# jac0626/Neighbor-Aware-Reinforcement-Learning-Fosters-Cooperation-in-Spatial-Public-Goods-Games-

Measured on AMD Instinct MI355X. Metric: agent-steps/sec (L×L×iters×replicas) + achieved HBM GB/s, L=200, higher is better.
Workload: dtype f64

## Files before the change

neighbor-aware-reinforcement-learning-fosters-cooperation-in-spatial-public-goods-games-_amd/csrc/spgg_device.h:

```cpp
#pragma once

#include <hip/hip_runtime.h>

#include <stdint.h>

#include "spgg_abi.h"

namespace spgg {

#ifndef SPGG_BLOCK
#define SPGG_BLOCK 256
#endif
constexpr int kBlock = SPGG_BLOCK;
static_assert(kBlock == 256 || kBlock == 512, "SPGG_BLOCK must be 256 or 512");
constexpr int kWaves = kBlock / 64;

__device__ __forceinline__ int wrap(int x, int L) {
  while (x < 0) x += L;
  while (x >= L) x -= L;
  return x;
}

template <int CTRL>
__device__ __forceinline__ double dpp_f64(double x) {
// ... 50 lines not shown
    constexpr int h = CNT > 1 ? CNT / 2 : 1;
    if constexpr (MASK >= 16) {
      if constexpr (CNT > 1) {
#pragma unroll
        for (int i = 0; i < h; ++i) v[i] = swap_sum<MASK>(v[i], v[i + h]);
      } else {
        v[0] = swap_sum<MASK>(v[0], v[0]);
      }
    } else {
      if constexpr (CNT > 1) {
        const bool upper = (lane & MASK) != 0;
#pragma unroll
        for (int i = 0; i < h; ++i) {
          const T send = upper ? v[i] : v[i + h];
          const T keep = upper ? v[i + h] : v[i];
          v[i] = keep + partner<MASK>(send);
        }
      } else {
        v[0] += partner<MASK>(v[0]);
      }
    }
    transpose_level<(CNT > 1 ? CNT / 2 : 1), MASK / 2, K, T>(v, lane);
  }
}

template <int K>
__device__ __forceinline__ double block_reduce(double (&v)[K], double* lds) {
  static_assert(K >= 1 && K <= 64 && (K & (K - 1)) == 0, "K must be a power of two");
  transpose_level<K, 32, K, double>(v, threadIdx.x & 63);
  const int lane = threadIdx.x & 63, wave = threadIdx.x >> 6;
  constexpr int per = 64 / K;
  if ((lane & (per - 1)) == 0) lds[wave * K + lane / per] = v[0];
  __syncthreads();
  double tot = 0.0;
  if (threadIdx.x < K) {
#pragma unroll
    for (int w = 0; w < kWaves; ++w) tot += lds[w * K + threadIdx.x];
  }
  return tot;
}

__device__ __forceinline__ double uniform_f64(double x) {
  return __hiloint2double(__builtin_amdgcn_readfirstlane(__double2hiint(x)),
                          __builtin_amdgcn_readfirstlane(__double2loint(x)));
}
__device__ __forceinline__ uint64_t uniform_u64(uint64_t x) {
  return (uint64_t)(uint32_t)__builtin_amdgcn_readfirstlane((int)(x >> 32)) << 32 |
         (uint32_t)__builtin_amdgcn_readfirstlane((int)(uint32_t)x);
}

__device__ __forceinline__ double max_f64(double a, double b) {
  double r;
  asm("v_max_f64 %0, %1, %2" : "=v"(r) : "v"(a), "v"(b));
  return r;
}

template <int MASK>
__device__ __forceinline__ double swap_max(double x) {
  const int lo = __double2loint(x), hi = __double2hiint(x);
  const auto l = MASK == 32 ? __builtin_amdgcn_permlane32_swap(lo, lo, false, false)
                            : __builtin_amdgcn_permlane16_swap(lo, lo, false, false);
  const auto h = MASK == 32 ? __builtin_amdgcn_permlane32_swap(hi, hi, false, false)
                            : __builtin_amdgcn_permlane16_swap(hi, hi, false, false);
  return max_f64(__hiloint2double(h[0], l[0]), __hiloint2double(h[1], l[1]));
}

__device__ __forceinline__ double wave_max(double v) {
  v = swap_max<32>(v);
  v = swap_max<16>(v);
  v = max_f64(v, partner<8>(v));
  v = max_f64(v, partner<4>(v));
  v = max_f64(v, partner<2>(v));
  v = max_f64(v, partner<1>(v));
  return v;
}

__device__ __forceinline__ double mt_double(uint32_t a, uint32_t b) {
  return ((double)(a >> 5) * 67108864.0 + (double)(b >> 6)) / 9007199254740992.0;
}

__device__ __forceinline__ uint2 philox2x32_10(uint2 c, uint32_t k) {
#pragma unroll
  for (int r = 0; r < 10; ++r) {
    if (r) k += 0x9E3779B9u;
    const uint64_t p = (uint64_t)0xD256D193u * c.x;
    c = make_uint2((uint32_t)(p >> 32) ^ k ^ c.y, (uint32_t)p);
  }
  return c;
}

__host__ __device__ inline uint64_t u53_threshold(double thr) {
  return (uint64_t)__builtin_ceil(thr * 9007199254740992.0);
}

__device__ __forceinline__ uint2 philox_block(int idx, int t, uint32_t key) {
  return philox2x32_10(make_uint2((uint32_t)idx >> 1, (uint32_t)t), key);
}
__device__ __forceinline__ void philox_decide(uint32_t bits, uint64_t thr53, int* explore, int* rbit) {
  const uint32_t thr31 = (uint32_t)((thr53 + ((1ull << 22) - 1)) >> 22);
  *explore = (bits >> 1) < thr31 ? 1 : 0;
  *rbit = (int)(bits & 1u);
}
__device__ __forceinline__ void philox_draw(int idx, int t, uint32_t key, uint64_t thr53, int* explore,
                                            int* rbit) {
  const uint2 w = philox_block(idx, t, key);
  philox_decide((idx & 1) ? w.y : w.x, thr53, explore, rbit);
// ... 45 lines not shown
```

neighbor-aware-reinforcement-learning-fosters-cooperation-in-spatial-public-goods-games-_amd/csrc/spgg_kernels.hip:

```cpp
#include <hip/hip_runtime.h>

#include <algorithm>
#include <numeric>
#include <type_traits>
#include <cstdio>
#include <cstdlib>
#include <cstring>
#include <new>
#include <string>
#include <thread>
#include <vector>

#include "spgg_abi.h"
#include "spgg_test.h"
#include "spgg_device.h"
#include "spgg_mt.h"
#include "spgg_clusters.h"
#include "spgg_correlations.h"
#include "spgg_reputation.h"

using namespace spgg;

#ifndef SPGG_ABLATE
#define SPGG_ABLATE 0
// ... 340 lines not shown
  __device__ __forceinline__ void store(uint8_t* dst, int pitch, int h, uint8_t* dbit, int tid) {
    const int r0 = tid / DW, col = tid - (tid / DW) * DW;
    const int o0 = r0 * pitch + col * 4;
#pragma unroll
    for (int j = 0; j < J; ++j) {
      if (r0 < RPP && r0 + j * RPP < h) {
        const int o = o0 + j * RPP * pitch;
        *reinterpret_cast<uint32_t*>(dst + o) = buf[j];
        if (dbit) *reinterpret_cast<uint32_t*>(dbit + o) = buf[j] & 0x01010101u;
      }
    }
  }
};

__device__ __forceinline__ void build_plus_counts(uint8_t* pc, const uint8_t* d, int sw, int rows, int tid) {
  const int lane = tid & 63;
  const int wave = __builtin_amdgcn_readfirstlane(tid >> 6);
  for (int y = wave; y < rows; y += kWaves) {
    const uint8_t* p = d + y * sw + lane;
    const int cnt = p[1] + p[sw] + p[sw + 1] + p[sw + 2] + p[2 * sw + 1];
    pc[y * kPcPitch + lane] = (uint8_t)(cnt << 3);
  }
}

template <int DWPR>
__device__ __forceinline__ void build_plus_counts_dw(uint8_t* pc, const uint8_t* dplane, int sw, int rows,
                                                     int soff, int tid) {
  const uint32_t s0 = 8u * soff, s1 = s0 + 8u, s2 = s0 + 16u;
  const int swd = sw >> 2;
  for (int task = tid; task < rows * DWPR; task += kBlock) {
    const int y = task / DWPR, xd = task - (task / DWPR) * DWPR;
    const uint32_t* r0 = reinterpret_cast<const uint32_t*>(dplane) + y * swd + xd;
    const uint32_t a0 = r0[0], a1 = r0[1];
    const uint32_t b0 = r0[swd], b1 = r0[swd + 1];
    const uint32_t c0 = r0[2 * swd], c1 = r0[2 * swd + 1];
    const uint32_t cnt = __builtin_amdgcn_alignbit(a1, a0, s1) + __builtin_amdgcn_alignbit(b1, b0, s0) +
                         __builtin_amdgcn_alignbit(b1, b0, s1) + __builtin_amdgcn_alignbit(b1, b0, s2) +
                         __builtin_amdgcn_alignbit(c1, c0, s1);
    *reinterpret_cast<uint32_t*>(pc + y * kPcPitch + xd * 4) = cnt << 3;
  }
}

__device__ __forceinline__ void build_plus_counts_prev(uint8_t* pc, const uint8_t* s, int sw, int rows, int tid) {
  const int lane = tid & 63;
  const int wave = __builtin_amdgcn_readfirstlane(tid >> 6);
  for (int y = wave; y < rows; y += kWaves) {
    const uint8_t* p = s + y * sw + lane;
    const int cnt = ((p[1] >> 3) & 1) + ((p[sw] >> 3) & 1) + ((p[sw + 1] >> 3) & 1) + ((p[sw + 2] >> 3) & 1) +
                    ((p[2 * sw + 1] >> 3) & 1);
    pc[y * kPcPitch + lane] = (uint8_t)(cnt << 3);
  }
}
template <int DWPR>
__device__ __forceinline__ void build_plus_counts_prev_dw(uint8_t* pc, const uint8_t* splane, int sw, int rows,
                                                          int soff, int tid) {
  const uint32_t s0 = 8u * soff, s1 = s0 + 8u, s2 = s0 + 16u;
  const int swd = sw >> 2;
  constexpr uint32_t kB3 = 0x01010101u;
  for (int task = tid; task < rows * DWPR; task += kBlock) {
    const int y = task / DWPR, xd = task - (task / DWPR) * DWPR;
    const uint32_t* r0 = reinterpret_cast<const uint32_t*>(splane) + y * swd + xd;
    const uint32_t a0 = (r0[0] >> 3) & kB3, a1 = (r0[1] >> 3) & kB3;
    const uint32_t b0 = (r0[swd] >> 3) & kB3, b1 = (r0[swd + 1] >> 3) & kB3;
    const uint32_t c0 = (r0[2 * swd] >> 3) & kB3, c1 = (r0[2 * swd + 1] >> 3) & kB3;
    const uint32_t cnt = __builtin_amdgcn_alignbit(a1, a0, s1) + __builtin_amdgcn_alignbit(b1, b0, s0) +
                         __builtin_amdgcn_alignbit(b1, b0, s1) + __builtin_amdgcn_alignbit(b1, b0, s2) +
                         __builtin_amdgcn_alignbit(c1, c0, s1);
    *reinterpret_cast<uint32_t*>(pc + y * kPcPitch + xd * 4) = cnt << 3;
  }
}

#define T_AT(t, o) (*reinterpret_cast<const double*>((t) + (o)))
__device__ __forceinline__ double payoff_pc(const uint8_t* pc, int ry, int rx, const double* tb, double norm_min,
                                            double norm_den, double norm_rcp) {
  const uint8_t* p = pc + ry * kPcPitch + rx + 1;
  const char* t = reinterpret_cast<const char*>(tb);
  const uint32_t x0 = p[kPcPitch], x1 = p[0], x2 = p[2 * kPcPitch], x3 = p[kPcPitch - 1], x4 = p[kPcPitch + 1];
  double tot = T_AT(t, x0);
  tot = tot + T_AT(t, x1);
  tot = tot + T_AT(t, x2);
  tot = tot + T_AT(t, x3);
  tot = tot + T_AT(t, x4);
  return div_uniform(tot - norm_min, norm_den, norm_rcp);
}

#undef T_AT

__device__ __forceinline__ double rcp_diag(double x) {
  double r = __builtin_amdgcn_rcp(x);
  r = __builtin_fma(r, __builtin_fma(-x, r, 1.0), r);
  r = __builtin_fma(r, __builtin_fma(-x, r, 1.0), r);
  return r;
}

constexpr uint64_t stat_bytes(int a, int b, int c, int d, int e, int f, int g, int h) {
  return (uint64_t)(uint8_t)a | (uint64_t)(uint8_t)b << 8 | (uint64_t)(uint8_t)c << 16 | (uint64_t)(uint8_t)d << 24 |
         (uint64_t)(uint8_t)e << 32 | (uint64_t)(uint8_t)f << 40 | (uint64_t)(uint8_t)g << 48 |
         (uint64_t)(uint8_t)h << 56;
}


enum { ALG_Q = SPGG_ALG_QLEARNING, ALG_SARSA = SPGG_ALG_SARSA, ALG_ES = SPGG_ALG_EXPECTED_SARSA,
       ALG_DQ = SPGG_ALG_DOUBLE_Q };

__device__ __forceinline__ int greedy2(double v0, double v1) { return v0 >= v1 ? 0 : 1; }

__device__ __forceinline__ double mean2(double x, double y) { return (x + y) * 0.5; }

__device__ __forceinline__ double expected_q(double v0, double v1, double eps) {
  const double po = eps * 0.5;
  const double pgr = (1.0 - eps) + po;
  const int g = greedy2(v0, v1);
  return (g == 0 ? pgr : po) * v0 + (g == 1 ? pgr : po) * v1;
}

__device__ __forceinline__ int draw_bit(const TileArgs& a, int rep, int g, int p) {
  const uint32_t w = *at(a.draws, (uint32_t)(rep * a.draw_words + (g >> 5) * a.planes + p));
  return (int)((w >> (g & 31)) & 1u);
}

template <int RNG>
// ... 128 lines not shown
    qb[0] = e == 0 ? nq2 : y0; qb[1] = e == 1 ? nq2 : y1; qb[2] = e == 2 ? nq2 : y2; qb[3] = e == 3 ? nq2 : y3;
    *rn0 = sn ? q[2] : q[0];
    *rn1 = sn ? q[3] : q[1];
    return diag ? diag_td_dq(q, qb, e, sn, rew, pg) : 0.f;
  } else {
    const double o0 = so ? q[2] : q[0], o1 = so ? q[3] : q[1];
    const double v0 = sn ? q[2] : q[0], v1 = sn ? q[3] : q[1];
    const double qc = act ? o1 : o0;
    double target;
    if constexpr (ALG == ALG_Q) {
      target = max_f64(v0, v1);
    } else if constexpr (ALG == ALG_SARSA) {
      int ex, rbt;
      draw_pair<RNG>(a, rep, g, t, key, eps53, 1, &ex, &rbt);
      target = (ex ? rbt : greedy2(v0, v1)) ? v1 : v0;
    } else {
      target = expected_q(v0, v1, eps);
    }
    const double td = (rew + gamma * target) - qc;
    const double q1 = qc + alpha * td;
    const bool s1 = so != 0, a1 = act != 0;
    q[0] = (!s1 && !a1) ? q1 : q[0];
    q[1] = (!s1 && a1) ? q1 : q[1];
    q[2] = (s1 && !a1) ? q1 : q[2];
    q[3] = (s1 && a1) ? q1 : q[3];
    const double w0 = sn ? q[2] : q[0], w1 = sn ? q[3] : q[1];
    *rn0 = w0;
    *rn1 = w1;
    if (!diag) return 0.f;
    double target2;
    if constexpr (ALG == ALG_SARSA) {
      int ex, rbt;
      draw_pair<RNG>(a, rep, g, t, key, eps53, 2, &ex, &rbt);
      target2 = (ex ? rbt : greedy2(w0, w1)) ? w1 : w0;
    } else {
      target2 = ALG == ALG_ES ? expected_q(w0, w1, eps) : max_f64(w0, w1);
    }
    return (float)fabs(pg.diag_alpha * ((rew + dgamma * target2) - q1));
  }
}

template <bool M2>
__device__ __forceinline__ double prev_max_diff(const double* rew, int ca, int w) {
  const double r0 = rew[ca];
  constexpr int KN = M2 ? 12 : 4;
  const int nb[12] = {ca - w, ca + w, ca - 1, ca + 1, ca - 2 * w, ca + 2 * w, ca - 2, ca + 2,
                      ca - w - 1, ca - w + 1, ca + w - 1, ca + w + 1};
  double rw[KN];
#pragma unroll
  for (int k = 0; k < KN; ++k) rw[k] = rew[nb[k]];
  double m = rw[0];
#pragma unroll
  for (int k = 1; k < KN; ++k) m = max_f64(m, rw[k]);
  return max_f64(m - r0, 0.0);
}

template <int ALG, typename PT>
__device__ __forceinline__ float prev_diag_td(const double (&q)[4], const double (&qb)[ALG == ALG_DQ ? 4 : 1],
                                              int e, int sn, double rew, const PT& pg, double eps_prev) {
  if constexpr (ALG == ALG_DQ) {
    return diag_td_dq(q, qb, e, sn, rew, pg);
  } else {
    double w0, w1, o0, o1;
    select_row<0>(q, qb, sn, &w0, &w1);
    select_row<0>(q, qb, e >> 1, &o0, &o1);
    const double q1 = (e & 1) ? o1 : o0;
    const double target2 = ALG == ALG_ES ? expected_q(w0, w1, eps_prev) : max_f64(w0, w1);
    return (float)fabs(pg.diag_alpha * ((rew + pg.diag_gamma * target2) - q1));
  }
}


__device__ __forceinline__ double wave_sum(double v) {
  {
    const int lo = __double2loint(v), hi = __double2hiint(v);
    const auto l = __builtin_amdgcn_permlane32_swap(lo, lo, false, false);
    const auto h = __builtin_amdgcn_permlane32_swap(hi, hi, false, false);
    v = __hiloint2double(h[0], l[0]) + __hiloint2double(h[1], l[1]);
  }
  {
    const int lo = __double2loint(v), hi = __double2hiint(v);
    const auto l = __builtin_amdgcn_permlane16_swap(lo, lo, false, false);
    const auto h = __builtin_amdgcn_permlane16_swap(hi, hi, false, false);
    v = __hiloint2double(h[0], l[0]) + __hiloint2double(h[1], l[1]);
  }
  v += partner<8>(v);
  v += partner<4>(v);
  v += partner<2>(v);
  v += partner<1>(v);
  return v;
}

#ifndef SPGG_BAR_DEBUG
#define SPGG_BAR_DEBUG 0
#endif
constexpr uint32_t kBarrierPolls = 1u << 21;

__device__ __forceinline__ bool replica_barrier(const spgg_impl::PersistArgs& pa, int rep, int tile,
                                                int tiles_per_rep, uint32_t k,
                                                unsigned long long* arrive_stamp = nullptr) {
  __shared__ int bar_ok;
  asm volatile("s_waitcnt vmcnt(0)" ::: "memory");
  __syncthreads();
  if (arrive_stamp && threadIdx.x == 0) *arrive_stamp = __builtin_amdgcn_s_memrealtime();
  if (threadIdx.x < 64) {
    const int lane = threadIdx.x, S = pa.shards;
    uint32_t* ctr = pa.bar + (size_t)rep * S * spgg_impl::kBarWords;
    if (lane == 0)
      __hip_atomic_fetch_add(ctr + (tile % S) * spgg_impl::kBarWords, 1u, __ATOMIC_RELAXED,
                             __HIP_MEMORY_SCOPE_AGENT);
    const int j = lane < S ? lane : 0;
    const uint32_t want = (uint32_t)((tiles_per_rep - j + S - 1) / S) * (pa.base + k);
    bool ok = false;
    for (uint32_t poll = 0; poll < kBarrierPolls; ++poll) {
      const uint32_t have = __hip_atomic_load(ctr + j * spgg_impl::kBarWords, __ATOMIC_RELAXED,
                                              __HIP_MEMORY_SCOPE_AGENT);
      const uint32_t err = __hip_atomic_load(pa.err, __ATOMIC_RELAXED, __HIP_MEMORY_SCOPE_AGENT);
      if (__builtin_amdgcn_readfirstlane(err) != 0) break;
      if (__all((int32_t)(have - want) >= 0)) {
// ... 12 lines not shown
      if ((int32_t)(have - want) < 0)
        printf("spgg barrier: rep %d tile %d k %u shard %d have %u want %u base %u\n", rep, tile, k, j, have, want,
               pa.base);
    }
#endif
    if (lane == 0) bar_ok = ok ? 1 : 0;
  }
  __syncthreads();
  return bar_ok != 0;
}

#ifndef SPGG_STAMPS
#define SPGG_STAMPS 0
#endif
#if SPGG_STAMPS
#ifndef SPGG_STAMP_T
#define SPGG_STAMP_T 30
#endif
constexpr int kStampWG = 8192, kStampSlots = 12;
__device__ unsigned long long spgg_stamps[kStampWG * kStampSlots];
#define STAMP(k)                                                                            \
  do {                                                                                      \
    if (t == SPGG_STAMP_T && tid == 0 && stamp_id < kStampWG)                               \
      spgg_stamps[stamp_id * kStampSlots + (k)] = __builtin_amdgcn_s_memrealtime();         \
  } while (0)
#else
#define STAMP(k) \
  do {           \
  } while (0)
#endif
constexpr int min_waves(bool m2, int rng, int twc, int alg) {
#ifdef SPGG_MIN_WAVES
  return SPGG_MIN_WAVES;
#else
#ifdef SPGG_MT_MIN_WAVES
  if (!m2 && rng == SPGG_RNG_MT19937 && twc > 0 && alg != SPGG_ALG_DOUBLE_Q) return SPGG_MT_MIN_WAVES;
#endif
  return (!m2 && rng == SPGG_RNG_PHILOX && twc > 0 && alg != SPGG_ALG_DOUBLE_Q) ? 4 : 1;
#endif
}

template <bool M2, bool AS, bool RQ, int RNG, int APT, int TWC, int ALG, bool PERSIST>
__device__ __forceinline__ void step_impl(const TileArgs& a0, const int t0, const int fin_only,
                                          const spgg_impl::PersistArgs& pa) {
  static_assert(!PERSIST || TWC > 0, "persistent launches use the compile-time-width kernels");
  using RT = RStore<RQ>;
  constexpr int HA = M2 ? 2 : 1;
  constexpr int HS = HA + 2;
  constexpr int QB = ALG == ALG_DQ ? 1 : 0;
  constexpr int QW = QB ? 8 : 4;
  constexpr int PF = spgg_impl::pf_of(ALG);
  constexpr bool RECOMP = ALG != ALG_SARSA && APT == spgg_impl::apt_of(ALG) && !(PERSIST && SPGG_PERSIST_NORECOMP);
  constexpr bool CARRY = PERSIST && !SPGG_PERSIST_NORECOMP;
  extern __shared__ __attribute__((aligned(16))) unsigned char smem[];

  const int total = a0.n_rep * a0.tiles_per_rep;
  const int per_xcd = (total + 7) / 8;
  const int logical = (blockIdx.x & 7) * per_xcd + (blockIdx.x >> 3);
  if (logical >= total) return;
  if (SPGG_ABLATE & 64) return;
  const int lrep = logical / a0.tiles_per_rep;
  const int tile = logical - lrep * a0.tiles_per_rep;
  const int rep = a0.rep_stride > 1 ? (int)(((uint32_t)lrep * (uint32_t)a0.rep_stride) % (uint32_t)a0.n_rep) : lrep;
#if SPGG_STAMPS
  const int stamp_id = (int)a0.params[rep].stream_id * a0.tiles_per_rep + tile;
#endif

  const int L = a0.L, n = a0.n;
  const bool tiny = TWC ? false : L < 8;
  const int tyi = tile / a0.tiles_x, txi = tile - (tile / a0.tiles_x) * a0.tiles_x;
  const int y0 = tyi * a0.TH, x0 = txi * a0.TW;
  const int th = min(a0.TH, L - y0), tw = TWC ? TWC : min(a0.TW, L - x0);
  constexpr bool DSTAGE = RNG != SPGG_RNG_PHILOX && TWC > 0;
  const LdsLayout ly = TWC ? lds_layout(TWC, a0.TH, HS, HA, (int)sizeof(RT), true, DSTAGE)
                           : lds_layout(tw, th, HS, HA, (int)sizeof(RT));
  double* tab = reinterpret_cast<double*>(smem);
  double* red = tab + 12;
  double* sRew = reinterpret_cast<double*>(smem + ly.off_Rew);
  RT* sR = reinterpret_cast<RT*>(smem + ly.off_R);
  RT* sRn = reinterpret_cast<RT*>(smem + ly.off_Rn);
  uint8_t* sS = smem + ly.off_S;
  uint8_t* sD = smem + ly.off_D;
  uint8_t* sA = smem + ly.off_A;
  uint8_t* sPC = smem + ly.off_PC;
  uint8_t* sPP = smem + ly.bytes;
  uint32_t* sDR = reinterpret_cast<uint32_t*>(smem + ly.off_DR);
  uint2* sDP = reinterpret_cast<uint2*>(smem + ly.off_DP);
  const size_t rb = (size_t)rep * n;
  double* Qr = a0.Q + rb * QW;
  double* mdr = a0.md + rb;
  float* atdr = a0.atd + rb;
  const int aw = tw + 2 * HA, ah = th + 2 * HA;

  int rc[APT];
  unsigned vbits = 0;
  double q[APT][4];
  double qb[APT][QB ? 4 : 1];
  double md_own[APT];
  float atd_own[APT];
  const int n_own = th * tw;
  const uint32_t g00 = (uint32_t)(y0 * L + x0);
  auto agent_of = [&](int rcu) { return g00 + __umul24((uint32_t)(rcu >> 16), (uint32_t)L) + ((rcu >> 8) & 0xff); };
  bool stored = false;
  int t = t0;
  for (;; ++t) {
  TileArgs a = a0;
  if constexpr (PERSIST) {
    const int cur = (t - 1) & 1, nxt = t & 1;
    a.S_in = pa.S[cur];
    a.S_out = pa.S[nxt];
    a.R_in = pa.R[cur];
    a.R_out = pa.R[nxt];
    a.pub_in = pa.pub[cur];
    a.pub_out = pa.pub[nxt];
    if (pa.draws0) a.draws = pa.draws0 + (size_t)((t - 1) % pa.draw_slots) * pa.draw_stride;
  }
  const bool first = !PERSIST || t == t0;
  int tid = threadIdx.x;
  if constexpr (PERSIST) asm volatile("" : "+v"(tid));
  const uint8_t* Sin = a.S_in + rb;
  uint8_t* Sout = a.S_out + rb;
  const RT* Rin = reinterpret_cast<const RT*>(a.R_in) + rb;
  RT* Rout = reinterpret_cast<RT*>(a.R_out) + rb;
  const bool pending = t > 1;
  STAMP(0);
#if SPGG_PRIO
  if constexpr (!PERSIST) __builtin_amdgcn_s_setprio(SPGG_PRIO);
#endif
#if SPGG_STAMPS
  if (t == SPGG_STAMP_T && tid == 0 && stamp_id < kStampWG) {
    unsigned hw, xcc;
    asm volatile("s_getreg_b32 %0, hwreg(HW_REG_HW_ID)" : "=s"(hw));
    asm volatile("s_getreg_b32 %0, hwreg(HW_REG_XCC_ID)" : "=s"(xcc));
    spgg_stamps[stamp_id * kStampSlots + 8] = hw;
    spgg_stamps[stamp_id * kStampSlots + 9] = xcc;
  }
#endif

  if (!first) {
#pragma unroll
    for (int u = 0; u < APT; ++u) rc[u] &= ~0xff;
  } else {
    const int dr = kBlock / tw, dc = kBlock - (kBlock / tw) * tw;
    int r = tid / tw, c = tid - (tid / tw) * tw;
#pragma unroll
    for (int u = 0; u < APT; ++u) {
      const int k = tid + u * kBlock;
      const bool own = k < n_own;
      rc[u] = own ? (r << 16) | (c << 8) : (TWC ? (tid & 1) << 8 : 0);
      vbits |= own ? 1u << u : 0u;
      const uint32_t g = own ? g00 + __umul24((uint32_t)r, (uint32_t)L) + (uint32_t)c : g00 + (TWC ? (tid & 1) : 0);
      if (SPGG_ABLATE & 512) {
#pragma unroll
        for (int k = 0; k < 4; ++k) q[u][k] = (double)((g + k) & 15) * 1e-3;
        if constexpr (QB) for (int k = 0; k < 4; ++k) qb[u][QB ? k : 0] = q[u][k];
        md_own[u] = 0.0;
        atd_own[u] = 0.f;
      } else {
        load_q<QB>(Qr, (uint32_t)n, g, q[u], qb[u]);
      }
      r += dr;
      c += dc;
      if (c >= tw) {
        c -= tw;
        ++r;
      }
    }
  }
  constexpr int RP = spgg_impl::ring_per_thread(M2);
  const int ring = aw * ah - n_own;
  int2 re[RP];
  {
    const int2* rtab = a.ring + (size_t)tile * a.ring_max;
#pragma unroll
    for (int j = 0; j < RP; ++j) re[j] = *at(rtab, (uint32_t)min(tid + j * kBlock, ring - 1));
  }
  constexpr int JRR = (25 + 2 * HA + kWaves - 1) / kWaves;
  constexpr int JSF = spgg_impl::js_of(M2), JRF = spgg_impl::jr_of();
  constexpr int DWS = (TWC + 2 * HS + 3 + 3) / 4, DWR = (TWC + 2 * HA + 3 + 3) / 4;
  constexpr int JSD = (25 + 2 * HS + kBlock / DWS - 1) / (kBlock / DWS);
  constexpr int JRD = (25 + 2 * HA + kBlock / DWR - 1) / (kBlock / DWR);
  const int soffS = TWC ? ((x0 - HS) & 3) : 0, soffR = TWC && RQ ? ((x0 - HA) & 3) : 0;
  uint8_t* sSv = sS + soffS;
  uint8_t* sDv = sD + soffS;
  RT* sRv = sR + soffR;
  DwordWindow<JSD, DWS> winS;
  DwordWindow<JRD, DWR> winRd;
  RowWindow<JRR, TWC + 2 * HA, RT> winR;
  if constexpr (TWC > 0) {
    winS.template load<PERSIST>(Sin, th + 2 * HS, y0 - HS, (x0 - HS) & ~3, L, tid);
    if constexpr (!AS) {
      if constexpr (RQ) winRd.template load<PERSIST>(Rin, ah, y0 - HA, (x0 - HA) & ~3, L, tid);
      else winR.template load<PERSIST>(Rin, ah, y0 - HA, x0 - HA, L, tid);
    }
  }

  if (!(SPGG_ABLATE & 512) && !RECOMP && (first || !CARRY)) {
    const bool ni_rec = __builtin_amdgcn_readfirstlane((int)(a.params[rep].kappa != 0.0)) != 0;
#pragma unroll
    for (int u = 0; u < APT; ++u) {
      const uint32_t g = ni_rec ? agent_of(rc[u]) : 0u;
// ... 3 lines not shown
  }
  const uint32_t xA = wrap_once(x0 - HA, L);
  const int a_len = min(aw, L - (int)xA);
  uint32_t dw0 = 0, dw1 = 0;
  if constexpr (DSTAGE) {
    const int i = min(tid, ah * kDrawSlots - 1), ry = i / kDrawSlots, sl = i - ry * kDrawSlots;
    const uint32_t gy = wrap_once(y0 - HA + ry, L);
    const uint32_t grp = min((gy * (uint32_t)L + (sl < 3 ? xA : 0u)) / 32u + (uint32_t)(sl % 3),
                             (uint32_t)(a.draw_words / a.planes - 1));
    const uint32_t wi = (uint32_t)rep * a.draw_words + grp * a.planes;
    dw0 = *at(a.draws, wi);
    dw1 = *at(a.draws, wi + 1);
  }
  const int st = first ? a.stop_iter[rep] : 0;
  const bool dead = st != 0 && st < t;
  const spgg_rep_params& pg = a.params[rep];
  __shared__ spgg_rep_params hps;
  static_assert(sizeof(spgg_rep_params) % 8 == 0, "spgg_rep_params: whole 8-byte words");
  constexpr int kParamWords = (int)(sizeof(spgg_rep_params) / 8);
  constexpr int kPayWord = (int)(offsetof(spgg_rep_params, pay_c) / 8);
  const uint64_t pword = *at(reinterpret_cast<const uint64_t*>(&pg),
                             (uint32_t)(tid < kParamWords ? tid
                                        : tid < kParamWords + 6 ? kPayWord + 5 - (tid - kParamWords)
                                        : kPayWord + 17 - min(tid - kParamWords, 11)));
  const spgg_rep_params& hp = hps;
  const double kappa = pg.kappa, w_p = pg.w_p, w_rep = pg.w_rep;
  const size_t stripe_len = (size_t)a.slots * SPGG_NSTAT;
  const double* rrow = a.stats + (size_t)rep * a.stripes * stripe_len;
  double* srow = a.stats + ((size_t)rep * a.stripes + tile % a.stripes) * stripe_len;
  bool stop_now = false;
  double gmax_prev = 0.0;
  if constexpr (PERSIST) {
    const int lane = tid & 63, k = lane < a.stripes ? lane : 0;
    const double ncv = hload<true>(rrow + k * stripe_len + (size_t)t * SPGG_NSTAT + SPGG_ST_NCOOP);
    const double gmv = pending ? hload<true>(rrow + k * stripe_len + (size_t)(t - 1) * SPGG_NSTAT + SPGG_ST_GMAX) : 0.0;
    const double nc = uniform_f64(wave_sum(lane < a.stripes ? ncv : 0.0));
    stop_now = (nc == 0.0) || (nc == (double)n);
    gmax_prev = uniform_f64(max_f64(wave_max(gmv), 0.0));
  } else {
    if (!fin_only) {
      double nc = 0.0;
      for (int k = 0; k < a.stripes; ++k) nc += rrow[k * stripe_len + (size_t)t * SPGG_NSTAT + SPGG_ST_NCOOP];
      stop_now = (nc == 0.0) || (nc == (double)n);
    }
    if (pending)
      for (int k = 0; k < a.stripes; ++k)
        gmax_prev = fmax(gmax_prev, rrow[k * stripe_len + (size_t)(t - 1) * SPGG_NSTAT + SPGG_ST_GMAX]);
  }
  const bool acting = !fin_only && !stop_now;
  const double lam_den = uniform_f64(pending ? gmax_prev + pg.lambda_eps : 1.0);
  const double lam_rcp = uniform_f64(1.0 / lam_den);
  const double eps_t = a.eps[(size_t)rep * a.slots + t];
  const double eps_prev = ALG == ALG_ES && pending ? a.eps[(size_t)rep * a.slots + t - 1] : 0.0;
  const uint64_t eps53 = uniform_u64(u53_threshold(eps_t));
  const uint32_t pkey = (uint32_t)pg.seed ^ (uint32_t)(pg.seed >> 32) * 0x85EBCA6Bu ^
                        (uint32_t)pg.stream_id * 0xC2B2AE35u;

  if (tid < kParamWords) reinterpret_cast<uint64_t*>(&hps)[tid] = pword;
  else if (tid < kParamWords + 12) reinterpret_cast<uint64_t*>(tab)[tid - kParamWords] = pword;
  if constexpr (TWC > 0) {
    winS.store(sS, ly.sw, th + 2 * HS, sD, tid);
    if constexpr (!AS) {
      if constexpr (RQ) winRd.store(reinterpret_cast<uint8_t*>(sR), ly.aw, ah, nullptr, tid);
      else winR.template store<(TWC + 2 * HS + 6) / 4 * 4>(sR, ah, nullptr, tid);
    }
  } else {
    stage_region<JSF>(sS, ly.sw, Sin, th + 2 * HS, tw + 2 * HS, y0 - HS, x0 - HS, L, tiny, sD);
    if (!AS) stage_region<JRF>(sR, ly.aw, Rin, ah, aw, y0 - HA, x0 - HA, L, tiny);
  }
  if constexpr (DSTAGE) {
    if (tid < ah * kDrawSlots) {
      sDR[tid * 2] = dw0;
      sDR[tid * 2 + 1] = dw1;
    }
  }
  if (dead) return;
  if (stop_now && tile == 0 && tid == 0) a.stop_iter[rep] = t;
  double rv[RP][PF];
  {
    const double* pin = a.pub_in + (size_t)rep * a.tiles_per_rep * PF * a.PB;
#pragma unroll
    for (int j = 0; j < RP; ++j)
#pragma unroll
      for (int f = 0; f < PF; ++f) rv[j][f] = hload<PERSIST>(at(pin, (uint32_t)(re[j].y + f * a.PB)));
  }
  __syncthreads();
  STAMP(1);
#if SPGG_PRIO
  if constexpr (!PERSIST) __builtin_amdgcn_s_setprio(0);
#endif
  if (SPGG_ABLATE & 128) {
#pragma unroll
    for (int u = 0; u < APT; ++u) {
      const int r = rc[u] >> 16, c = (rc[u] >> 8) & 0xff;
      store_q<QB>(Qr, (uint32_t)n, agent_of(rc[u]), q[u], qb[u]);
      if (!RECOMP) {
        *at(mdr, agent_of(rc[u])) = md_own[u];
        *at(atdr, agent_of(rc[u])) = atd_own[u];
      }
      *at(Sout, agent_of(rc[u])) = sSv[(r + HS) * ly.sw + (c + HS)];
      if (!AS) *at(Rout, agent_of(rc[u])) = sRv[(r + HA) * ly.aw + (c + HA)];
    }
    return;
  }
  if (!fin_only) {
    if constexpr (TWC > 0) build_plus_counts_dw<(TWC + 2 * HA + 2 + 3) / 4>(sPC, sD, ly.sw, ah + 2, soffS, tid);
    else build_plus_counts(sPC, sDv, ly.sw, ah + 2, tid);
  }
  const bool rec_prev = RECOMP && pending && kappa != 0.0;
  if (rec_prev) {
    if constexpr (TWC > 0) build_plus_counts_prev_dw<(TWC + 2 * HA + 2 + 3) / 4>(sPP, sS, ly.sw, ah + 2, soffS, tid);
    else build_plus_counts_prev(sPP, sSv, ly.sw, ah + 2, tid);
    __syncthreads();
    const int dr = kBlock / aw, dc = kBlock - (kBlock / aw) * aw;
    int ry = tid / aw, rx = tid - (tid / aw) * aw;
    for (int k = tid; k < aw * ah; k += kBlock) {
      const uint8_t b = sSv[(ry + (HS - HA)) * ly.sw + (rx + (HS - HA))];
      const double P = payoff_pc(sPP, ry, rx, tab + (((b >> 3) & 1) ? 6 : 0), hp.norm_min, hp.norm_den, hp.norm_rcp);
      const double rr = (b & 1) ? 0.0 : 0.5;
      const double wpp = w_p * P, wrr = w_rep * rr;
      sRew[ry * ly.aw + rx] = wpp + wrr;
      ry += dr;
      rx += dc;
      if (rx >= aw) {
        rx -= aw;
        ++ry;
      }
    }
    __syncthreads();
  }
  if constexpr (DSTAGE) {
    if (!fin_only && tid < ah * 2) {
      const int ry = tid >> 1, r0 = (tid & 1) * 32;
      const uint32_t gyL = wrap_once(y0 - HA + ry, L) * (uint32_t)L;
      const int offA = (int)((gyL + xA) & 31u), offB = (int)(gyL & 31u);
      const uint32_t* W = sDR + ry * kDrawSlots * 2;
      auto bits32 = [&](int slot0, int bitpos, int p) {
        const int w = bitpos >> 5;
        const uint32_t lo = W[(slot0 + min(w, 2)) * 2 + p], hi = W[(slot0 + min(w + 1, 2)) * 2 + p];
        return __builtin_amdgcn_alignbit(hi, lo, (uint32_t)(bitpos & 31));
      };
      uint32_t out[2] = {0u, 0u};
#pragma unroll
      for (int p = 0; p < 2; ++p) {
        if (r0 < a_len) out[p] = bits32(0, offA + r0, p);
        if (a_len < r0 + 32) {
          const int rs = max(r0, a_len), sh = rs - r0;
          const uint32_t mB = ~0u << sh;
          out[p] = (out[p] & ~mB) | ((bits32(3, offB + rs - a_len, p) << sh) & mB);
        }
      }
      sDP[ry * 2 + (r0 >> 5)] = make_uint2(out[0], out[1]);
    }
  }

  float pct_t1 = 0.f;
  uint32_t ni_rows = 0;
  {
    double v[8];
    float pct = 0.f;
#pragma unroll
    for (int k = 0; k < 8; ++k) v[k] = 0.0;
    uint8_t sb[APT];
#pragma unroll
    for (int u = 0; u < APT; ++u) {
      const int r = rc[u] >> 16, c = (rc[u] >> 8) & 0xff;
      sb[u] = sSv[(r + HS) * ly.sw + (c + HS)];
      rc[u] |= (AS ? 0 : ((sb[u] >> 4) & 1) << 1) | ((sb[u] & 1) << 3);
    }
    if (pending) {
#pragma unroll
      for (int u = 0; u < APT; ++u) {
        const double vmu = (vbits >> u) & 1 ? 1.0 : 0.0;
        const uint8_t b = sb[u];
        const int e = pending_entry(b);
        if (kappa != 0.0) {
          double mdp;
          float atdv;
          if constexpr (RECOMP) {
            const int r = rc[u] >> 16, c = (rc[u] >> 8) & 0xff;
            const int ca = (r + HA) * ly.aw + (c + HA);
            mdp = prev_max_diff<M2>(sRew, ca, ly.aw);
            atdv = prev_diag_td<ALG>(q[u], qb[u], e, (b >> 4) & 1, sRew[ca], hp, eps_prev);
          } else {
            mdp = md_own[u];
            atdv = atd_own[u];
          }
          const double nu = pending_nu(b, mdp, kappa, lam_den, lam_rcp);
#pragma unroll
          for (int k = 0; k < 4; ++k) {
            const double m = e == k ? 1.0 : 0.0;
            q[u][k] = __builtin_fma(m, nu, q[u][k]);
            if constexpr (QB) qb[u][k] = __builtin_fma(m, nu, qb[u][QB ? k : 0]);
          }
          ni_rows |= (1u << (e >> 1)) << (2 * u);
          const float anu = fabsf((float)nu);
          pct = (SPGG_ABLATE & 32768) ? 0.f : __builtin_fmaf(anu * __builtin_amdgcn_rcpf((atdv + anu) + 1e-8f), (float)vmu, pct);
        }
        const double cm = ((b >> 3) & 1) ? 0.0 : vmu;
#pragma unroll
        for (int e2 = 0; e2 < 4; ++e2) {
          const double qv = QB ? mean2(q[u][e2], qb[u][QB ? e2 : 0]) : q[u][e2];
          v[e2] = __builtin_fma(qv, vmu, v[e2]);
          v[4 + e2] = __builtin_fma(qv, cm, v[4 + e2]);
        }
      }
    }
    wave_partials<8>(v, red, 0, tid);
    pct_t1 = pct;
  }
  if (!acting) {
#pragma unroll
    for (int u = 0; u < APT; ++u) store_q<QB>(Qr, (uint32_t)n, agent_of(rc[u]), q[u], qb[u]);
    stored = true;
  }
  double* sRec = reinterpret_cast<double*>(smem + ly.bytes);
#pragma unroll
  for (int j = 0; j < RP; ++j) {
    const int k = tid + j * kBlock;
    if (k < ring) {
#pragma unroll
      for (int f = 0; f < PF; ++f) sRec[k * PF + f] = rv[j][f];
    }
  }
  STAMP(2);
  __syncthreads();

  uint32_t cw0 = 0, cw1 = 0;
  constexpr bool PAIRED = RNG == SPGG_RNG_PHILOX && TWC > 0 && APT % 2 == 0 && !(SPGG_ABLATE & 1);
  uint32_t pbits[APT];
  {
    double va[4] = {0.0, 0.0, 0.0, 0.0};
    RVal<RQ> rsum = 0;
#pragma unroll
    for (int u = 0; u < APT; ++u) {
      if (fin_only) continue;
      const int r = rc[u] >> 16, c = (rc[u] >> 8) & 0xff;
      const uint32_t one = (vbits >> u) & 1;
      const double vmu = one ? 1.0 : 0.0;
      const int cs = (r + HS) * ly.sw + (c + HS);
      const int ca = (r + HA) * ly.aw + (c + HA);
      const int s_t = (rc[u] >> 3) & 1;
      const double P = payoff_pc(sPC, r + HA, c + HA, tab + (s_t ? 6 : 0), hp.norm_min, hp.norm_den,
                                 hp.norm_rcp);
      const RVal<RQ> r_t = AS ? hload<PERSIST>(at(Rin, agent_of(rc[u]))) : sRv[ca];
      if constexpr (RQ) rsum += one ? r_t : 0;
      else rsum = __builtin_fma(r_t, vmu, rsum);
      if (!acting) continue;
      if constexpr (PAIRED) {
        if (u % 2 == 0) {
          const bool odd = tid & 1;
          const uint2 w = philox_block((int)agent_of(rc[odd ? u + 1 : u]), t, pkey);
          const uint32_t keep = odd ? w.y : w.x, recv = partner<1>(odd ? w.x : w.y);
          pbits[u] = odd ? recv : keep;
          pbits[u + 1] = odd ? keep : recv;
        }
      }
      int so;
      if constexpr (AS) so = s_t == 0 ? 1 : 0;
      else so = (rc[u] >> 1) & 1;
      int ex, rbt;
      if constexpr (PAIRED) philox_decide(pbits[u], eps53, &ex, &rbt);
      else if constexpr (DSTAGE) staged_draw(sDP, r + HA, c + HA, &ex, &rbt);
      else draw_pair<RNG>(a, rep, agent_of(rc[u]), t, pkey, eps53, 0, &ex, &rbt);
      double qs0, qs1;
      select_row<QB>(q[u], qb[u], so, &qs0, &qs1);
      const int act = ex ? rbt : greedy2(qs0, qs1);
      const RVal<RQ> rn = rep_next<RQ>(r_t, act, hp);
      const double rr = act == 0 ? 0.5 : 0.0;
      const double wpp = w_p * P, wrr = w_rep * rr;
      const double rew = wpp + wrr;
      sA[ca] = (uint8_t)act;
      sRn[ca] = (RT)rn;
      sRew[ca] = rew;
      rc[u] |= act | (AS ? so << 1 : 0);
      cw0 += (s_t == 0 && act == 1) ? one : 0u;
      cw1 += act == 0 ? one : 0u;
      const double am = act ? 0.0 : vmu;
      va[1] = __builtin_fma(rew, am, va[1]);
      if (w_rep != 0.0) va[2] = __builtin_fma(fabs(wrr) * rcp_diag(fabs(rew) + 1e-9), am, va[2]);
    }
    va[0] = (double)rsum;
    va[3] = (double)pct_t1;
    if (!(SPGG_ABLATE & (8 | 65536))) wave_partials<4>(va, red, 16, tid);
  }
  STAMP(3);

  if (acting && !(SPGG_ABLATE & 4)) {
#pragma unroll
    for (int j = 0; j < RP; ++j) {
      const int k = tid + j * kBlock;
      if (k >= ring) break;
      int ay, ax;
      spgg_impl::ring_cell(k, th, tw, HA, &ay, &ax);
      const int g = re[j].x;
      const int cs = (ay + (HS - HA)) * ly.sw + (ax + (HS - HA));
      const uint8_t b = sSv[cs];
      const double* rec = sRec + k * PF;
      double v0 = rec[0], v1 = rec[1], w0 = 0.0, w1 = 0.0;
      if constexpr (QB) {
        w0 = rec[QB ? 2 : 0];
        w1 = rec[QB ? 3 : 0];
      }
      if (pending && kappa != 0.0) {
        const int e = pending_entry(b);
        if ((e >> 1) == ((b >> 4) & 1)) {
          const double nu = pending_nu(b, rec[PF - 1], kappa, lam_den, lam_rcp);
          if (e & 1) v1 = v1 + nu; else v0 = v0 + nu;
          if constexpr (QB) {
            if (e & 1) w1 = w1 + nu; else w0 = w0 + nu;
          }
        }
      }
      const double P = payoff_pc(sPC, ay, ax, tab + ((b & 1) ? 6 : 0), hp.norm_min, hp.norm_den, hp.norm_rcp);
      const RVal<RQ> r_t = AS ? RVal<RQ>(0) : RVal<RQ>(sRv[ay * ly.aw + ax]);
      int ex, rbt;
      if constexpr (DSTAGE) staged_draw(sDP, ay, ax, &ex, &rbt);
      else draw_pair<RNG>(a, rep, g, t, pkey, eps53, 0, &ex, &rbt);
      const int act = ex ? rbt : (QB ? greedy2(mean2(v0, w0), mean2(v1, w1)) : greedy2(v0, v1));
      const RVal<RQ> rn = rep_next<RQ>(r_t, act, hp);
      const double rr = act == 0 ? 0.5 : 0.0;
      const int ca = ay * ly.aw + ax;
      sA[ca] = (uint8_t)act;
      sRn[ca] = (RT)rn;
      const double wpp = w_p * P, wrr = w_rep * rr;
      sRew[ca] = wpp + wrr;
    }
  }
  __syncthreads();
  STAMP(4);

  double bmax = 0.0;
  uint32_t gcn = 0, nmd2 = 0;
  if (acting) {
    double* pout = a.pub_out + (size_t)(rep * a.tiles_per_rep + tile) * PF * a.PB;
    const uint64_t bsw = *at(reinterpret_cast<const uint64_t*>(a.ring + (size_t)a.tiles_per_rep * a.ring_max),
                             (uint32_t)(((th != a.TH ? 2 : 0) + (tw != a.TW ? 1 : 0)) * kBlock + tid));
    const bool ni_on = __builtin_amdgcn_readfirstlane((int)(kappa != 0.0)) != 0;
    const bool diag_on = ni_on && !RECOMP;
#pragma unroll
    for (int u = 0; u < APT; ++u) {
      const int r = rc[u] >> 16, c = (rc[u] >> 8) & 0xff;
      const int ca = (r + HA) * ly.aw + (c + HA);
      const uint32_t one = (vbits >> u) & 1;
      const int act = rc[u] & 1, so = (rc[u] >> 1) & 1;
      const double rew = sRew[ca];
      int sn;
      if constexpr (AS) sn = act == 0 ? 1 : 0;
      else sn = rep_state_lds<M2>(sRn, ca, ly.aw);
      double rn0, rn1;
      const float atd = td_update<ALG, RNG>(a, hp, rep, agent_of(rc[u]), t, pkey, eps_t, eps53, diag_on, rew, so,
                                            act, sn, q[u], qb[u], &rn0, &rn1);
      if constexpr (CARRY) atd_own[u] = atd;
      else if (diag_on && !(SPGG_ABLATE & (256 | 2048))) *at(atdr, agent_of(rc[u])) = atd;
      if (!PERSIST && !(SPGG_ABLATE & 2048)) {
        uint32_t rows = ((ni_rows >> (2 * u)) & 3u) | (1u << so);
#if SPGG_QSTORE == 1
        rows = 3u;
#elif SPGG_QSTORE == 2
        rows |= (uint32_t)__shfl_xor((int)rows, 1);
        rows |= (uint32_t)__shfl_xor((int)rows, 2);
        rows |= (uint32_t)__shfl_xor((int)rows, 4);
#elif SPGG_QSTORE == 3
        if constexpr (TWC > 0 && TWC % 2 == 0) rows |= partner<1>(rows);
#elif SPGG_QSTORE == 4
        if constexpr (TWC > 0 && TWC % 8 == 0) {
          rows |= partner<1>(rows);
          rows |= partner<2>(rows);
          rows |= partner<4>(rows);
        }
#endif
        store_q<QB>(Qr, (uint32_t)n, agent_of(rc[u]), q[u], qb[u], rows);
      }
      const int w = ly.aw;
      constexpr int KN = M2 ? 12 : 4;
      const int nb[12] = {ca - w, ca + w, ca - 1, ca + 1,
                          ca - 2 * w, ca + 2 * w, ca - 2, ca + 2,
                          ca - w - 1, ca - w + 1, ca + w - 1, ca + w + 1};
      double rw[KN];
      int an[KN];
#pragma unroll
      for (int kk = 0; kk < KN; ++kk) {
        rw[kk] = sRew[nb[kk]];
        an[kk] = sA[nb[kk]];
      }
      double md = rw[0] - rew;
      int abest = an[0], ks = 0;
#pragma unroll
      for (int kk = 1; kk < KN; ++kk) {
        const double d = rw[kk] - rew;
        const bool better = d > md;
        md = max_f64(md, d);
        abest = better ? an[kk] : abest;
        if constexpr (M2) ks = better ? kk : ks;
      }
      const int dp = abest == act ? 1 : 0;
      const double mdp = max_f64(md, 0.0);
      bmax = max_f64(bmax, mdp);
      if constexpr (CARRY) md_own[u] = mdp;
      else if (ni_on && !RECOMP && !(SPGG_ABLATE & (2048 | 8192))) *at(mdr, agent_of(rc[u])) = mdp;
      hstore<PERSIST>(at(Sout, agent_of(rc[u])), (uint8_t)((rc[u] & 0xff) | (dp << 2) | (sn << 4)));
      hstore<PERSIST>(at(Rout, agent_of(rc[u])), (RT)sRn[ca]);
      const int bslot = (int)(int16_t)(uint16_t)(bsw >> (16 * u));
      if (bslot >= 0) {
        double* rec = pout + bslot;
        hstore<PERSIST>(rec, rn0);
        hstore<PERSIST>(rec + a.PB, rn1);
        if constexpr (QB) {
          hstore<PERSIST>(rec + 2 * a.PB, sn ? qb[u][QB ? 2 : 0] : qb[u][0]);
          hstore<PERSIST>(rec + 3 * a.PB, sn ? qb[u][QB ? 3 : 0] : qb[u][QB ? 1 : 0]);
        }
        if (ni_on) hstore<PERSIST>(rec + (PF - 1) * a.PB, mdp);
      }
      const int nd = act + an[0] + an[1] + an[2] + an[3];
      gcn += one << (4 * nd);
      if (md > 0.0) {
        cw1 += one << 16;
        if (M2 && ks >= 4) nmd2 += one;
      }
    }
  }
  STAMP(5);
  if (!(SPGG_ABLATE & (8 | 131072))) {
    uint32_t cw[8] = {cw0,
                      cw1,
                      nmd2 | ((gcn & 0xfu) << 16),
                      ((gcn >> 4) & 0xfu) | (((gcn >> 8) & 0xfu) << 16),
                      ((gcn >> 12) & 0xfu) | (((gcn >> 16) & 0xfu) << 16),
                      (gcn >> 20) & 0xfu,
                      0u,
                      0u};
    wave_partials<8>(cw, red, 24, tid);
  }
  {
    const double wm = wave_max(bmax);
    if ((tid & 63) == 0) red[(tid >> 6) * 64 + 12] = wm;
  }
  if (SPGG_ABLATE & 16) {
    if (tid == 0 && tile == 0 && acting) srow[(size_t)(t + 1) * SPGG_NSTAT] = n / 2;
    return;
  }
  __syncthreads();
  STAMP(6);

  if ((SPGG_ABLATE & (8 | 131072)) && tid == 0 && tile == 0 && acting) srow[(size_t)(t + 1) * SPGG_NSTAT] = n / 2;
  if ((SPGG_ABLATE & 16392) == 16392 && tid == 40 && acting) {
    double bm = 0.0;
#pragma unroll
    for (int w = 0; w < kWaves; ++w) bm = max_f64(bm, red[w * 64 + 12]);
    if (bm > 0.0)
      atomicMax(reinterpret_cast<unsigned long long*>(&srow[(size_t)t * SPGG_NSTAT + SPGG_ST_GMAX]),
// ... 696 lines not shown
  const int i = idx / L, j = idx - (idx / L) * L;
  const int im1 = wrap(i - 1, L), ip1 = wrap(i + 1, L), im2 = wrap(i - 2, L), ip2 = wrap(i + 2, L);
  const int jm1 = wrap(j - 1, L), jp1 = wrap(j + 1, L), jm2 = wrap(j - 2, L), jp2 = wrap(j + 2, L);
#define CO(r, c) ((s[(r) * L + (c)] & 1) ? 0 : 1)
  Cells13 c;
  c.c00 = CO(i, j); c.cm0 = CO(im1, j); c.cp0 = CO(ip1, j); c.c0m = CO(i, jm1); c.c0p = CO(i, jp1);
  c.cmm = CO(im1, jm1); c.cmp = CO(im1, jp1); c.cpm = CO(ip1, jm1); c.cpp = CO(ip1, jp1);
  c.cM0 = CO(im2, j); c.cP0 = CO(ip2, j); c.c0M = CO(i, jm2); c.c0P = CO(i, jp2);
#undef CO
  out[(size_t)rep * n + idx] = payoff13(c, tab, params[rep].norm_min, params[rep].norm_den, params[rep].norm_rcp);
}

}

struct spgg_ctx {
  spgg_config cfg{};
  spgg_buffers buf{};
  bool bound = false;
  bool params_set = false;
  int gen_chunk = 8, draw_slots = 16, snap_slots = 25;
  int chains = 1, per_chain = 8, jump_levels = 0;
  uint32_t* d_parts[2] = {nullptr, nullptr};
  uint32_t* d_keybuf[2] = {nullptr, nullptr};
  uint32_t* d_run_pos0 = nullptr;
  uint32_t* d_polys = nullptr;
  int64_t draw_words = 0;
  hipStream_t gen_stream = nullptr;
  bool own_gen_stream = false;
  hipEvent_t gen_done[2] = {nullptr, nullptr}, step_done[2] = {nullptr, nullptr}, gen_idle = nullptr;
  hipEvent_t caller_ready = nullptr;
  uint32_t* d_err = nullptr;
  volatile uint32_t* h_err = nullptr;
  int gen_upto = 0;
  std::vector<spgg_rep_params> params_host;
  bool params_moved = false;
  spgg_rep_params* d_params = nullptr;
  int2* d_ring = nullptr;
  int ring_max = 0;
  int n = 0;
  int TW = 0, TH = 0, tiles_x = 0, tiles_per_rep = 0, apt = 4, PB = 0;
  int stripes = 1;
  int rep_stride = 1;
  size_t lds_bytes = 0;
  bool persist = false;
  int persist_capacity = 0;
  uint32_t* d_bar = nullptr;
  uint32_t bar_base = 0;
  std::string err;
};

namespace {

int twc_of(const spgg_config& cfg, int TW, int TH) {
  if (TW == 40 && cfg.L % 40 == 0 && cfg.L >= 120 && TH <= 25) return 40;
  if (TW == 20 && cfg.L % 20 == 0 && cfg.L >= 60 && TH <= 25 && cfg.algorithm != SPGG_ALG_DOUBLE_Q) return 20;
  return 0;
}

thread_local std::string g_create_err;

int fail(spgg_ctx* c, int code, const std::string& msg) {
  if (c) c->err = msg;
  return code;
}

int create_fail(int code, const std::string& msg) {
  g_create_err = msg;
  return code;
}

int hip_check(spgg_ctx* c, hipError_t e, const char* what) {
  if (e == hipSuccess) return SPGG_OK;
  return fail(c, SPGG_E_HIP, std::string(what) + ": " + hipGetErrorString(e));
}

const char* tuning_env(const char* name) {
  const char* on = getenv("SPGG_TUNING");
  return on && !strcmp(on, "1") ? getenv(name) : nullptr;
}

constexpr long long kSmallBatchTiles = 128;
constexpr long long kTwoPerThreadTiles = 800;

constexpr double kGenRateMargin = 2.0;

void choose_mt_chains(spgg_ctx* c) {
  const spgg_config& cfg = c->cfg;
  const long long W = draw_mt_words(c->n, draw_planes(cfg.algorithm));
  int chains = 1, per = 8;
  const long long batch = cfg.batch_reps > 0 ? cfg.batch_reps : cfg.n_rep;
  if (W >= 4096) {
    const double gen_ns = W / 227.0 * 200.0;
    const double step_ns = std::max(8000.0, (double)batch * c->n * 0.015);
    const double need = kGenRateMargin * gen_ns / step_ns;
    while (chains < 256 && chains < need) chains *= 2;
    if (chains > 1)
      per = (int)std::max((1000000 + W - 1) / W, (long long)((128 + chains - 1) / chains));
    const double rec = draw_words_of(c->n, cfg.algorithm) * 4.0 * batch;
    while (chains > 1 && 2.0 * chains * per * rec > 512e6) {
      if (per > 1) per = std::max(1, per / 2);
      else chains /= 2;
    }
  }
  if (const char* e = tuning_env("SPGG_MT_CHAINS")) {
    int v = atoi(e), p2 = 1;
    while (p2 < 256 && p2 < v) p2 *= 2;
    chains = W >= 624 ? std::max(1, p2) : 1;
// ... 894 lines not shown
```

Measured before the change: 85.41 billion.

## Fuse current/previous plus-count builds and trim per-agent ownership and max ops

Merges the current and previous plus-count LDS passes into one pass that masks two bit planes at once, and drops the separate derived-plane store. It also treats the first APT-1 agent slots as always owned on 40-wide tiles, with a host-side guard added to twc_of, and replaces max with zero by an inline-constant v_max_f64. Further changes compute the Philox epsilon threshold directly in 31-bit form and apply the pending Q update as a select rather than four FMAs. The main risk is correctness: the ownership assumption relies on the new guard, and the select-based update assumes qe matches the entry being replaced.

```diff
diff --git a/neighbor-aware-reinforcement-learning-fosters-cooperation-in-spatial-public-goods-games-_amd/csrc/spgg_device.h b/neighbor-aware-reinforcement-learning-fosters-cooperation-in-spatial-public-goods-games-_amd/csrc/spgg_device.h
--- a/neighbor-aware-reinforcement-learning-fosters-cooperation-in-spatial-public-goods-games-_amd/csrc/spgg_device.h
+++ b/neighbor-aware-reinforcement-learning-fosters-cooperation-in-spatial-public-goods-games-_amd/csrc/spgg_device.h
@@ -126,6 +126,12 @@
 __device__ __forceinline__ double max_f64(double a, double b) {
   double r;
   asm("v_max_f64 %0, %1, %2" : "=v"(r) : "v"(a), "v"(b));
+  return r;
+}
+
+__device__ __forceinline__ double max0_f64(double a) {
+  double r;
+  asm("v_max_f64 %0, %1, 0" : "=v"(r) : "v"(a));
   return r;
 }
 
diff --git a/neighbor-aware-reinforcement-learning-fosters-cooperation-in-spatial-public-goods-games-_amd/csrc/spgg_kernels.hip b/neighbor-aware-reinforcement-learning-fosters-cooperation-in-spatial-public-goods-games-_amd/csrc/spgg_kernels.hip
--- a/neighbor-aware-reinforcement-learning-fosters-cooperation-in-spatial-public-goods-games-_amd/csrc/spgg_kernels.hip
+++ b/neighbor-aware-reinforcement-learning-fosters-cooperation-in-spatial-public-goods-games-_amd/csrc/spgg_kernels.hip
@@ -416,21 +416,22 @@
   }
 }
 template <int DWPR>
-__device__ __forceinline__ void build_plus_counts_prev_dw(uint8_t* pc, const uint8_t* splane, int sw, int rows,
-                                                          int soff, int tid) {
+__device__ __forceinline__ void build_plus_counts_both_dw(uint8_t* pc, uint8_t* pp, const uint8_t* splane, int sw,
+                                                          int rows, int soff, bool prev, int tid) {
   const uint32_t s0 = 8u * soff, s1 = s0 + 8u, s2 = s0 + 16u;
   const int swd = sw >> 2;
-  constexpr uint32_t kB3 = 0x01010101u;
+  constexpr uint32_t kB03 = 0x09090909u;
   for (int task = tid; task < rows * DWPR; task += kBlock) {
     const int y = task / DWPR, xd = task - (task / DWPR) * DWPR;
     const uint32_t* r0 = reinterpret_cast<const uint32_t*>(splane) + y * swd + xd;
-    const uint32_t a0 = (r0[0] >> 3) & kB3, a1 = (r0[1] >> 3) & kB3;
-    const uint32_t b0 = (r0[swd] >> 3) & kB3, b1 = (r0[swd + 1] >> 3) & kB3;
-    const uint32_t c0 = (r0[2 * swd] >> 3) & kB3, c1 = (r0[2 * swd + 1] >> 3) & kB3;
+    const uint32_t a0 = r0[0] & kB03, a1 = r0[1] & kB03;
+    const uint32_t b0 = r0[swd] & kB03, b1 = r0[swd + 1] & kB03;
+    const uint32_t c0 = r0[2 * swd] & kB03, c1 = r0[2 * swd + 1] & kB03;
     const uint32_t cnt = __builtin_amdgcn_alignbit(a1, a0, s1) + __builtin_amdgcn_alignbit(b1, b0, s0) +
                          __builtin_amdgcn_alignbit(b1, b0, s1) + __builtin_amdgcn_alignbit(b1, b0, s2) +
                          __builtin_amdgcn_alignbit(c1, c0, s1);
-    *reinterpret_cast<uint32_t*>(pc + y * kPcPitch + xd * 4) = cnt << 3;
+    *reinterpret_cast<uint32_t*>(pc + y * kPcPitch + xd * 4) = (cnt & 0x07070707u) << 3;
+    if (prev) *reinterpret_cast<uint32_t*>(pp + y * kPcPitch + xd * 4) = cnt & 0x38383838u;
   }
 }
 
@@ -665,12 +666,13 @@
   double m = rw[0];
 #pragma unroll
   for (int k = 1; k < KN; ++k) m = max_f64(m, rw[k]);
-  return max_f64(m - r0, 0.0);
+  return max0_f64(m - r0);
 }
 
 template <int ALG, typename PT>
 __device__ __forceinline__ float prev_diag_td(const double (&q)[4], const double (&qb)[ALG == ALG_DQ ? 4 : 1],
-                                              int e, int sn, double rew, const PT& pg, double eps_prev) {
+                                              int e, int sn, double rew, const PT& pg, double eps_prev,
+                                              double* qe) {
   if constexpr (ALG == ALG_DQ) {
     return diag_td_dq(q, qb, e, sn, rew, pg);
   } else {
@@ -678,6 +680,7 @@
     select_row<0>(q, qb, sn, &w0, &w1);
     select_row<0>(q, qb, e >> 1, &o0, &o1);
     const double q1 = (e & 1) ? o1 : o0;
+    *qe = q1;
     const double target2 = ALG == ALG_ES ? expected_q(w0, w1, eps_prev) : max_f64(w0, w1);
     return (float)fabs(pg.diag_alpha * ((rew + pg.diag_gamma * target2) - q1));
   }
@@ -796,6 +799,7 @@
   constexpr int PF = spgg_impl::pf_of(ALG);
   constexpr bool RECOMP = ALG != ALG_SARSA && APT == spgg_impl::apt_of(ALG) && !(PERSIST && SPGG_PERSIST_NORECOMP);
   constexpr bool CARRY = PERSIST && !SPGG_PERSIST_NORECOMP;
+  constexpr bool BOTH = RECOMP && TWC > 0;
   extern __shared__ __attribute__((aligned(16))) unsigned char smem[];
 
   const int total = a0.n_rep * a0.tiles_per_rep;
@@ -838,6 +842,8 @@
 
   int rc[APT];
   unsigned vbits = 0;
+  constexpr int NFULL = (TWC == 40 && APT == spgg_impl::apt_of(ALG)) ? APT - 1 : 0;
+  auto owned = [&](int u) -> uint32_t { return u < NFULL ? 1u : (vbits >> u) & 1u; };
   double q[APT][4];
   double qb[APT][QB ? 4 : 1];
   double md_own[APT];
@@ -890,7 +896,7 @@
 #pragma unroll
     for (int u = 0; u < APT; ++u) {
       const int k = tid + u * kBlock;
-      const bool own = k < n_own;
+      const bool own = u < NFULL || k < n_own;
       rc[u] = own ? (r << 16) | (c << 8) : (TWC ? (tid & 1) << 8 : 0);
       vbits |= own ? 1u << u : 0u;
       const uint32_t g = own ? g00 + __umul24((uint32_t)r, (uint32_t)L) + (uint32_t)c : g00 + (TWC ? (tid & 1) : 0);
@@ -1000,14 +1006,17 @@
   const double lam_rcp = uniform_f64(1.0 / lam_den);
   const double eps_t = a.eps[(size_t)rep * a.slots + t];
   const double eps_prev = ALG == ALG_ES && pending ? a.eps[(size_t)rep * a.slots + t - 1] : 0.0;
-  const uint64_t eps53 = uniform_u64(u53_threshold(eps_t));
+  const uint64_t eps53 = RNG == SPGG_RNG_PHILOX
+                             ? (uint64_t)(uint32_t)__builtin_amdgcn_readfirstlane(
+                                   (int)(uint32_t)__builtin_ceil(eps_t * 2147483648.0)) << 22
+                             : uniform_u64(u53_threshold(eps_t));
   const uint32_t pkey = (uint32_t)pg.seed ^ (uint32_t)(pg.seed >> 32) * 0x85EBCA6Bu ^
                         (uint32_t)pg.stream_id * 0xC2B2AE35u;
 
   if (tid < kParamWords) reinterpret_cast<uint64_t*>(&hps)[tid] = pword;
   else if (tid < kParamWords + 12) reinterpret_cast<uint64_t*>(tab)[tid - kParamWords] = pword;
   if constexpr (TWC > 0) {
-    winS.store(sS, ly.sw, th + 2 * HS, sD, tid);
+    winS.store(sS, ly.sw, th + 2 * HS, BOTH ? nullptr : sD, tid);
     if constexpr (!AS) {
       if constexpr (RQ) winRd.store(reinterpret_cast<uint8_t*>(sR), ly.aw, ah, nullptr, tid);
       else winR.template store<(TWC + 2 * HS + 6) / 4 * 4>(sR, ah, nullptr, tid);
@@ -1051,14 +1060,16 @@
     }
     return;
   }
-  if (!fin_only) {
+  const bool rec_prev = RECOMP && pending && kappa != 0.0;
+  if constexpr (BOTH) {
+    if (!fin_only || rec_prev)
+      build_plus_counts_both_dw<(TWC + 2 * HA + 2 + 3) / 4>(sPC, sPP, sS, ly.sw, ah + 2, soffS, rec_prev, tid);
+  } else if (!fin_only) {
     if constexpr (TWC > 0) build_plus_counts_dw<(TWC + 2 * HA + 2 + 3) / 4>(sPC, sD, ly.sw, ah + 2, soffS, tid);
     else build_plus_counts(sPC, sDv, ly.sw, ah + 2, tid);
   }
-  const bool rec_prev = RECOMP && pending && kappa != 0.0;
   if (rec_prev) {
-    if constexpr (TWC > 0) build_plus_counts_prev_dw<(TWC + 2 * HA + 2 + 3) / 4>(sPP, sS, ly.sw, ah + 2, soffS, tid);
-    else build_plus_counts_prev(sPP, sSv, ly.sw, ah + 2, tid);
+    if constexpr (!BOTH) build_plus_counts_prev(sPP, sSv, ly.sw, ah + 2, tid);
     __syncthreads();
     const int dr = kBlock / aw, dc = kBlock - (kBlock / aw) * aw;
     int ry = tid / aw, rx = tid - (tid / aw) * aw;
@@ -1119,27 +1130,36 @@
     if (pending) {
 #pragma unroll
       for (int u = 0; u < APT; ++u) {
-        const double vmu = (vbits >> u) & 1 ? 1.0 : 0.0;
+        const double vmu = owned(u) ? 1.0 : 0.0;
         const uint8_t b = sb[u];
         const int e = pending_entry(b);
         if (kappa != 0.0) {
-          double mdp;
+          double mdp, qe = 0.0;
           float atdv;
           if constexpr (RECOMP) {
             const int r = rc[u] >> 16, c = (rc[u] >> 8) & 0xff;
             const int ca = (r + HA) * ly.aw + (c + HA);
             mdp = prev_max_diff<M2>(sRew, ca, ly.aw);
-            atdv = prev_diag_td<ALG>(q[u], qb[u], e, (b >> 4) & 1, sRew[ca], hp, eps_prev);
+            atdv = prev_diag_td<ALG>(q[u], qb[u], e, (b >> 4) & 1, sRew[ca], hp, eps_prev, &qe);
           } else {
             mdp = md_own[u];
             atdv = atd_own[u];
           }
           const double nu = pending_nu(b, mdp, kappa, lam_den, lam_rcp);
-#pragma unroll
-          for (int k = 0; k < 4; ++k) {
-            const double m = e == k ? 1.0 : 0.0;
-            q[u][k] = __builtin_fma(m, nu, q[u][k]);
-            if constexpr (QB) qb[u][k] = __builtin_fma(m, nu, qb[u][QB ? k : 0]);
+          if constexpr (RECOMP && !QB) {
+            const double x = qe + nu;
+            const bool s1 = (e & 2) != 0, a1 = (e & 1) != 0;
+            q[u][0] = (!s1 && !a1) ? x : q[u][0];
+            q[u][1] = (!s1 && a1) ? x : q[u][1];
+            q[u][2] = (s1 && !a1) ? x : q[u][2];
+            q[u][3] = (s1 && a1) ? x : q[u][3];
+          } else {
+#pragma unroll
+            for (int k = 0; k < 4; ++k) {
+              const double m = e == k ? 1.0 : 0.0;
+              q[u][k] = __builtin_fma(m, nu, q[u][k]);
+              if constexpr (QB) qb[u][k] = __builtin_fma(m, nu, qb[u][QB ? k : 0]);
+            }
           }
           ni_rows |= (1u << (e >> 1)) << (2 * u);
           const float anu = fabsf((float)nu);
@@ -1184,7 +1204,7 @@
     for (int u = 0; u < APT; ++u) {
       if (fin_only) continue;
       const int r = rc[u] >> 16, c = (rc[u] >> 8) & 0xff;
-      const uint32_t one = (vbits >> u) & 1;
+      const uint32_t one = owned(u);
       const double vmu = one ? 1.0 : 0.0;
       const int cs = (r + HS) * ly.sw + (c + HS);
       const int ca = (r + HA) * ly.aw + (c + HA);
@@ -1290,7 +1310,7 @@
     for (int u = 0; u < APT; ++u) {
       const int r = rc[u] >> 16, c = (rc[u] >> 8) & 0xff;
       const int ca = (r + HA) * ly.aw + (c + HA);
-      const uint32_t one = (vbits >> u) & 1;
+      const uint32_t one = owned(u);
       const int act = rc[u] & 1, so = (rc[u] >> 1) & 1;
       const double rew = sRew[ca];
       int sn;
@@ -1343,8 +1363,8 @@
         if constexpr (M2) ks = better ? kk : ks;
       }
       const int dp = abest == act ? 1 : 0;
-      const double mdp = max_f64(md, 0.0);
-      bmax = max_f64(bmax, mdp);
+      const double mdp = max0_f64(md);
+      bmax = u == 0 ? mdp : max_f64(bmax, mdp);
       if constexpr (CARRY) md_own[u] = mdp;
       else if (ni_on && !RECOMP && !(SPGG_ABLATE & (2048 | 8192))) *at(mdr, agent_of(rc[u])) = mdp;
       hstore<PERSIST>(at(Sout, agent_of(rc[u])), (uint8_t)((rc[u] & 0xff) | (dp << 2) | (sn << 4)));
@@ -2147,7 +2167,10 @@
 namespace {
 
 int twc_of(const spgg_config& cfg, int TW, int TH) {
-  if (TW == 40 && cfg.L % 40 == 0 && cfg.L >= 120 && TH <= 25) return 40;
+  const int th_min = cfg.L % TH ? cfg.L % TH : TH;
+  if (TW == 40 && cfg.L % 40 == 0 && cfg.L >= 120 && TH <= 25 &&
+      th_min * 40 > (spgg_impl::apt_of(cfg.algorithm) - 1) * kBlock)
+    return 40;
   if (TW == 20 && cfg.L % 20 == 0 && cfg.L >= 60 && TH <= 25 && cfg.algorithm != SPGG_ALG_DOUBLE_Q) return 20;
   return 0;
 }
```

New measurement: 87.80 billion, median of 6. +2.8%, better.
